# ScuffleCloud/SVT-AV1-mirror

Measured on AMD Instinct MI355X. Metric: open-loop ME 64x64 superblocks/sec + achieved HBM GB/s, 4K preset-8, higher is better.
Workload: dtype u8

## Files before the change

### svt-av1-mirror_amd/csrc/svtme_me_common.h

```cpp
#pragma once
#include <hip/hip_runtime.h>
#include <stdint.h>

#include "svtme_device.h"

#define U32MAX 0xFFFFFFFFu

namespace svtme {

template <typename S, typename T>
__device__ __forceinline__ uint32_t sfld_(const S &obj, const T &f) {
    static_assert(sizeof(T) <= 2 && alignof(S) >= 4, "sfld_: a byte / halfword of a dword-aligned struct");
    const uint32_t off = (uint32_t)((const char *)&f - (const char *)&obj);
    const uint32_t v   = ((const uint32_t *)&obj)[off >> 2] >> (8 * (off & 3));
    return sizeof(T) == 1 ? (v & 0xFFu) : (v & 0xFFFFu);
}
#define SF(obj, field) ::svtme::sfld_((obj), (obj).field)
__device__ __forceinline__ bool tl_or_l0(const svtme_job &j, int l) { return j.temporal_layer_index > 0 || l == 0; }
__device__ __forceinline__ bool slot_valid(uint32_t vmask, int s) { return s >= 0 && s < 8 && ((vmask >> s) & 1u); }
__device__ __forceinline__ uint32_t valid_mask(const svtme_job &job) {
    uint32_t m = 0;
#pragma unroll
    for (int s = 0; s < 8; s++)
        if ((s >> 2) < job.num_lists && (s & 3) < job.num_refs[s >> 2])
            m |= 1u << s;
    return m;
}

#define DPP_ROW_SHR(n) (0x110 + (n))
#define DPP_ROW_BCAST15 0x142
#define DPP_ROW_BCAST31 0x143

template <int CTRL, int RM = 0xF>
__device__ __forceinline__ uint32_t dpp_or(uint32_t v, uint32_t id) {
    return (uint32_t)__builtin_amdgcn_update_dpp((int)id, (int)v, CTRL, RM, 0xF, false);
}
template <typename F>
__device__ __forceinline__ uint32_t wave_scan32(uint32_t v, uint32_t id, F f) {
    v = f(v, dpp_or<DPP_ROW_SHR(1)>(v, id));
    v = f(v, dpp_or<DPP_ROW_SHR(2)>(v, id));
    v = f(v, dpp_or<DPP_ROW_SHR(4)>(v, id));
    v = f(v, dpp_or<DPP_ROW_SHR(8)>(v, id));
    v = f(v, dpp_or<DPP_ROW_BCAST15, 0xA>(v, id));
    v = f(v, dpp_or<DPP_ROW_BCAST31, 0xC>(v, id));
    return v;
}
__device__ __forceinline__ uint32_t lane63(uint32_t v) { return (uint32_t)__builtin_amdgcn_readlane((int)v, 63); }

__device__ __forceinline__ unsigned long long wave_min_u64(unsigned long long v) {
    auto step = [&](uint32_t tl, uint32_t th) {
        const unsigned long long t = ((unsigned long long)th << 32) | tl;
        v                          = t < v ? t : v;
    };
#define WMIN64(CTRL, RM)                                                                                              \
    step(dpp_or<CTRL, RM>((uint32_t)v, U32MAX), dpp_or<CTRL, RM>((uint32_t)(v >> 32), U32MAX))
    WMIN64(DPP_ROW_SHR(1), 0xF);
    WMIN64(DPP_ROW_SHR(2), 0xF);
    WMIN64(DPP_ROW_SHR(4), 0xF);
    WMIN64(DPP_ROW_SHR(8), 0xF);
    WMIN64(DPP_ROW_BCAST15, 0xA);
    WMIN64(DPP_ROW_BCAST31, 0xC);
#undef WMIN64
    return ((unsigned long long)lane63((uint32_t)(v >> 32)) << 32) | lane63((uint32_t)v);
}
__device__ __forceinline__ uint32_t wave_min_u32(uint32_t v) {
    return lane63(wave_scan32(v, U32MAX, [](uint32_t a, uint32_t b) { return a < b ? a : b; }));
}
__device__ __forceinline__ uint32_t wave_sum_u32(uint32_t v) {
    return lane63(wave_scan32(v, 0u, [](uint32_t a, uint32_t b) { return a + b; }));
}
__device__ __forceinline__ int wave_compact(bool pred, int *total) {
    const unsigned long long m = __ballot(pred);
    *total                     = __popcll(m);
    const int lane             = threadIdx.x & 63;
    const unsigned long long lt = lane ? (m & ((1ull << lane) - 1ull)) : 0ull;
    return __popcll(lt);
}

__device__ __forceinline__ int wave_incl_scan(int v) {
    return (int)wave_scan32((uint32_t)v, 0u, [](uint32_t a, uint32_t b) { return a + b; });
}

__device__ __forceinline__ uint32_t magic_u32(uint32_t d) { return 0xFFFFFFFFu / d + 1u; }
__device__ __forceinline__ int mdiv(int n, uint32_t m) { return m ? (int)__umulhi((uint32_t)n, m) : n; }

__device__ __forceinline__ uint32_t xcd_remap(uint32_t bid, uint32_t nwg) {
    const uint32_t xcd = bid & 7, q8 = nwg >> 3, r8 = nwg & 7;
    return (xcd < r8 ? xcd * (q8 + 1) : r8 * (q8 + 1) + (xcd - r8) * q8) + (bid >> 3);
}

#define UNI(x) __builtin_amdgcn_readfirstlane((int)(x))
__device__ __forceinline__ uint32_t rl32(uint32_t v, int l) { return (uint32_t)__builtin_amdgcn_readlane((int)v, l); }
__device__ __forceinline__ uint64_t rl64(uint64_t v, int l) {
    return ((uint64_t)rl32((uint32_t)(v >> 32), l) << 32) | rl32((uint32_t)v, l);
}

template <typename T>
__device__ __forceinline__ T *uni_ptr(T *p) {
    const uint64_t v  = (uint64_t)(uintptr_t)p;
    const uint32_t lo = __builtin_amdgcn_readfirstlane((uint32_t)v);
    const uint32_t hi = __builtin_amdgcn_readfirstlane((uint32_t)(v >> 32));
    return (T *)(uintptr_t)(((uint64_t)hi << 32) | lo);
}

__device__ __forceinline__ unsigned long long qsad(uint32_t lo, uint32_t hi, uint32_t s, unsigned long long a) {
    return __builtin_amdgcn_qsad_pk_u16_u8(((unsigned long long)hi << 32) | lo, s, a);
}
__device__ __forceinline__ void qsad_unpack(unsigned long long a, uint32_t acc[4]) {
    acc[0] += (uint32_t)a & 0xFFFFu;
    acc[1] += (uint32_t)a >> 16;
    acc[2] += (uint32_t)(a >> 32) & 0xFFFFu;
    acc[3] += (uint32_t)(a >> 48);
}

template <int CTRL, int RM = 0xF>
__device__ __forceinline__ uint32_t dpp_add(uint32_t v) {
    return v + (uint32_t)__builtin_amdgcn_update_dpp(0, (int)v, CTRL, RM, 0xF, false);
}

template <int CTRL, int RM = 0xF>
__device__ __forceinline__ uint32_t dpp_add2(uint32_t a, uint32_t b) {
    return a + (uint32_t)__builtin_amdgcn_update_dpp(0, (int)b, CTRL, RM, 0xF, false);
}

__device__ void prehme_area(const DevPlane &p, int16_t org_x, int16_t org_y, int16_t sa_w, int16_t sa_h, int16_t *oxo,
                            int16_t *oyo, int16_t *saw, int16_t *sah) {
    const int16_t pad_w = i16(p.pad - 1), pad_h = i16(p.pad - 1);
    const int16_t pw = i16(p.width), ph = i16(p.height);
    int16_t ox = -(int16_t)(sa_w >> 1);
    int16_t oy = -(int16_t)(sa_h >> 1);
    ox   = ((org_x + ox) < -pad_w) ? i16(-pad_w - org_x) : ox;
    sa_w = ((org_x + ox) < -pad_w) ? i16(sa_w - (-pad_w - (org_x + ox))) : sa_w;
    ox   = ((org_x + ox) > pw - 1) ? i16(ox - ((org_x + ox) - (pw - 1))) : ox;
    sa_w = ((org_x + ox + sa_w) > pw) ? i16(max(1, sa_w - ((org_x + ox + sa_w) - pw))) : sa_w;
    oy   = ((org_y + oy) < -pad_h) ? i16(-pad_h - org_y) : oy;
    sa_h = ((org_y + oy) < -pad_h) ? i16(sa_h - (-pad_h - (org_y + oy))) : sa_h;
    oy   = ((org_y + oy) > ph - 1) ? i16(oy - ((org_y + oy) - (ph - 1))) : oy;
    sa_h = (org_y + oy + sa_h > ph) ? i16(max(1, sa_h - ((org_y + oy + sa_h) - ph))) : sa_h;
    *oxo = ox, *oyo = oy, *saw = sa_w, *sah = sa_h;
}

__device__ void hme_l0_rect(const svtme_controls &c, const DevPlane &p, int16_t org_x, int16_t org_y, int16_t sa_w,
                            int16_t sa_h, int sr_w, int sr_h, int16_t *oxo, int16_t *oyo, int16_t *saw,
                            int16_t *sah) {
    sa_w = i16((sa_w + 7) & ~0x07);
    const int16_t pad_w = i16(p.pad - 1), pad_h = i16(p.pad - 1);
    const int16_t pw = i16(p.width), ph = i16(p.height);
    const int16_t xd = i16(sa_w * sr_w), yd = i16(sa_h * sr_h);
    int16_t ox = i16(-(int16_t)((sa_w * c.num_hme_sa_w) >> 1) + xd);
    int16_t oy = i16(-(int16_t)((sa_h * c.num_hme_sa_h) >> 1) + yd);
    if ((org_x + ox) < -pad_w) {
        ox   = i16(-pad_w - org_x);
        sa_w = i16(sa_w - (-pad_w - (org_x + ox)));
    }
    if ((org_x + ox) > pw - 1)
        ox = i16(ox - ((org_x + ox) - (pw - 1)));
    if ((org_x + ox + sa_w) > pw)
        sa_w = i16(max(1, sa_w - ((org_x + ox + sa_w) - pw)));
    sa_w = (sa_w < 8) ? sa_w : i16(sa_w & ~0x07);
    if ((org_y + oy) < -pad_h) {
        oy   = i16(-pad_h - org_y);
        sa_h = i16(sa_h - (-pad_h - (org_y + oy)));
    }
    if ((org_y + oy) > ph - 1)
        oy = i16(oy - ((org_y + oy) - (ph - 1)));
    if ((org_y + oy + sa_h) > ph)
        sa_h = i16(max(1, sa_h - ((org_y + oy + sa_h) - ph)));
// ... 61 lines not shown
```

### svt-av1-mirror_amd/csrc/svtme_stages.hip

```cpp
#include <hip/hip_ext.h>
#include <cstdlib>
#include <type_traits>

#include "svtme_launch.h"
#include "svtme_me_common.h"

namespace svtme {


#define STAGE_A_BUF_DW 1024
#define STAGE_B_BUF_DW 640

template <int ND, typename P>
__device__ __forceinline__ void rows_qsad(P rp, int bstride_dw, const uint8_t *src, int src_stride,
                                          int k0, int k1, uint32_t acc[4]) {
    constexpr int CH = 64 / ND;
    for (int kc = k0; kc < k1; kc += CH) {
        const int ke         = min(k1, kc + CH);
        unsigned long long a = 0;
#pragma unroll 2
        for (int k = kc; k < ke; k++) {
            const P rd         = rp + k * bstride_dw;
            const uint32_t *sd = (const uint32_t *)(src + k * src_stride);
            uint32_t d[ND + 1];
// ... 887 lines not shown
        if (tk) {
            if (hk) {
                scx = cx;
                scy = cy;
            }
        } else {
            scx = 0;
            scy = 0;
        }
        if (s == k) {
            my_scx = scx, my_scy = scy, my_hs = cs;
        }
    }
    uint64_t hsad = U32MAX;
    if (valid)
        hsad = my_hs;
    uint32_t rdiv = 1;
    uint8_t dref  = s < 8 ? dref0 : 0;
    if (hme_on && !mctf) {
        if (prune && pth != 0xFFFFu) {
            const uint64_t best = wave_min_u64(s < 8 ? hsad : ~0ull);
            if (s < 8 && (s & 3) >= 1 && (hsad - best) * 100 > (pth * best))
                dref = 0;
        }
        if (sradj && s < 8) {
            if (absi(my_scx) <= mvlen && absi(my_scy) <= mvlen && hsad < stat_th)
                rdiv = stat_div;
            else if (hsad < low_th)
                rdiv = low_div;
        }
    }
    SlotCentre o;
    o.hme_sad    = hsad;
    o.zz         = s < 8 ? zz0 : U32MAX;
    o.reduce_div = rdiv;
    o.sc_x       = valid ? my_scx : 0;
    o.sc_y       = valid ? my_scy : 0;
    o.do_ref     = dref;
    return o;
}

#ifndef HME_STAMP
#define HME_STAMP(k)
#endif
#ifndef HME_STOP
#define HME_STOP(k)
#endif
#ifndef HME_SUB
#define HME_SUB(k)
#endif
#ifndef HME_WAVE
#define HME_WAVE(k)
#endif

#define HQ 2
#define HQ1 2
#define HQ16 2

typedef uint32_t u32x4a4 __attribute__((ext_vector_type(4), aligned(4)));
__device__ __forceinline__ u32x4a4 ldg4(const uint32_t *p) {
    typedef __attribute__((address_space(1))) const u32x4a4 gu4;
    return *(gu4 *)(uintptr_t)p;
}
__device__ __forceinline__ __amdgpu_buffer_rsrc_t plane_rsrc(const void *base) {
    return __builtin_amdgcn_make_buffer_rsrc(const_cast<void *>(base), 0, (int)0xFFFFFFFF, 0x00020000);
}
__device__ __forceinline__ u32x4a4 bld4(__amdgpu_buffer_rsrc_t r, uint32_t voff, uint32_t soff) {
    const auto v = __builtin_amdgcn_raw_buffer_load_b128(r, (int)voff, (int)soff, 0);
    u32x4a4 o;
    o.x = v[0], o.y = v[1], o.z = v[2], o.w = v[3];
    return o;
}
__device__ __forceinline__ uint4 sld4(const uint8_t *p) {
    typedef __attribute__((address_space(4))) const uint32_t cu32;
    cu32 *q = (cu32 *)(uintptr_t)p;
    return make_uint4(q[0], q[1], q[2], q[3]);
}
__device__ __forceinline__ unsigned long long qsad64(unsigned long long ref, uint32_t s, unsigned long long a) {
    return __builtin_amdgcn_qsad_pk_u16_u8(ref, s, a);
}
__device__ __forceinline__ unsigned long long pair(uint32_t lo, uint32_t hi) {
    return ((unsigned long long)hi << 32) | lo;
}

struct HSrch {
    const uint8_t *a0;
    int32_t item0;
    int16_t sa_w, ncols;
    int16_t cnt0, cnt1;
    int16_t ylast;
    uint32_t ncm;
    uint8_t sh, skip, id;
    uint8_t need;
    uint8_t tt;
};
struct HSrch1 {
    const uint8_t *a0;
    int32_t item0;
    uint32_t ncm;
    int16_t sa_w, ncols;
    uint8_t sh, id;
};


typedef uint32_t u32x2a4 __attribute__((ext_vector_type(2), aligned(4)));
struct Row8 {
    u32x4a4 lo;
    u32x2a4 hi;
};
__device__ __forceinline__ Row8 row8(const uint8_t *a0, int stride, int ro, int q0) {
    typedef __attribute__((address_space(1))) const u32x2a4 gu2;
    const uint32_t *rp = (const uint32_t *)(a0 + (ptrdiff_t)ro * stride) + q0;
    return Row8{ldg4(rp), *(gu2 *)(uintptr_t)(rp + 4)};
}

template <int T, bool FULLK = false>
__device__ __forceinline__ unsigned long long hme_tile16(const uint8_t *a0, int stride, int q0, int sh, int sa_w,
                                                         int yf, int tv, int ylast, int kh,
                                                         const uint32_t (&sr)[8][4]) {
    constexpr int NR = T + 7;
    kh = UNI(kh);
    unsigned long long acc[T][HQ16];
#pragma unroll
    for (int t = 0; t < T; t++)
#pragma unroll
        for (int qq = 0; qq < HQ16; qq++) acc[t][qq] = 0;
    Row8 buf[3];
    buf[0] = row8(a0, stride, min(yf, ylast), q0);
    buf[1] = row8(a0, stride, min(yf + 2, ylast), q0);
#pragma unroll
    for (int m = 0; m < NR; m++) {
        if (m + 2 < NR)
            buf[(m + 2) % 3] = row8(a0, stride, min(yf + 2 * (m + 2), ylast), q0);
        const Row8 &R = buf[m % 3];
        static_assert(HQ16 + 4 == 6, "Row8 holds 6 dwords");
        const uint32_t d[6] = {R.lo.x, R.lo.y, R.lo.z, R.lo.w, R.hi.x, R.hi.y};
        unsigned long long P[HQ16 + 3];
#pragma unroll
        for (int j = 0; j < HQ16 + 3; j++) P[j] = pair(d[j], d[j + 1]);
#pragma unroll
        for (int t = 0; t < T; t++) {
            const int k = m - t;
            if (k < 0 || k >= 8)
                continue;
            if (!FULLK && k >= kh)
                continue;
#pragma unroll
            for (int qq = 0; qq < HQ16; qq++)
#pragma unroll
                for (int j = 0; j < 4; j++) acc[t][qq] = qsad64(P[qq + j], sr[k][j], acc[t][qq]);
        }
    }
    uint32_t xo[HQ16][4];
#pragma unroll
    for (int qq = 0; qq < HQ16; qq++)
#pragma unroll
        for (int e = 0; e < 4; e++) {
            const int x = 4 * (q0 + qq) - sh + e;
            xo[qq][e]   = (x >= 0 && x < sa_w) ? (uint32_t)x : U32MAX;
        }
    unsigned long long best = ~0ull;
    uint32_t yk = (uint32_t)yf;
    asm volatile("" : "+v"(yk));
#pragma unroll
    for (int t = 0; t < T; t++) {
        uint32_t mt = U32MAX;
#pragma unroll
        for (int qq = 0; qq < HQ16; qq++) {
            const uint32_t lo = (uint32_t)acc[t][qq], hi = (uint32_t)(acc[t][qq] >> 32);
            const uint32_t k0 = (lo << 16) | xo[qq][0], k1 = (lo & 0xFFFF0000u) | xo[qq][1];
            const uint32_t k2 = (hi << 16) | xo[qq][2], k3 = (hi & 0xFFFF0000u) | xo[qq][3];
            mt = min_u32(mt, min_u32(min_u32(k0, k1), min_u32(k2, k3)));
        }
        if (t < tv && mt != U32MAX) {
            const unsigned long long kk = ((unsigned long long)(mt >> 16) << 32) |
                                          ((unsigned long long)(yk + 2 * t) << 16) | (mt & 0xFFFFu);
            best = kk < best ? kk : best;
        }
    }
    return best;
}

template <bool FULLK = false>
__device__ __forceinline__ unsigned long long hme_tile32q(const uint8_t *a0, int stride, int q0, int sh, int sa_w,
                                                          int y, int kh1, const uint8_t (*src)[32]) {
    const int g = threadIdx.x & 3;
    static_assert(HQ1 + 9 == 11, "L1 rows hold 11 dwords");
    typedef uint32_t u32x3a4 __attribute__((ext_vector_type(3), aligned(4)));
    typedef __attribute__((address_space(1))) const u32x3a4 gu3;
    struct Row11 {
        u32x4a4 a, b;
        u32x3a4 c;
    };
    auto ld = [&](int kk, Row11 &L) {
        const int k        = min(4 * g + kk, 15);
        const uint32_t *rp = (const uint32_t *)(a0 + (ptrdiff_t)(y + 2 * k) * stride) + q0;
        L.a = ldg4(rp), L.b = ldg4(rp + 4), L.c = *(gu3 *)(uintptr_t)(rp + 8);
    };
    Row11 L[2];
    ld(0, L[0]);
    unsigned long long acc[HQ1] = {};
#pragma unroll
    for (int kk = 0; kk < 4; kk++) {
        if (kk + 1 < 4)
            ld(kk + 1, L[(kk + 1) & 1]);
        const int k = min(4 * g + kk, 15);
        {
            const Row11 &R = L[kk & 1];
            const uint4 s0 = ((const uint4 *)src[k])[0], s1 = ((const uint4 *)src[k])[1];
            const uint32_t sv[8] = {s0.x, s0.y, s0.z, s0.w, s1.x, s1.y, s1.z, s1.w};
            uint32_t d[11] = {R.a.x, R.a.y, R.a.z, R.a.w, R.b.x, R.b.y, R.b.z, R.b.w, R.c.x, R.c.y, R.c.z};
#pragma unroll
            for (int j = 0; j < HQ1 + 8; j++) d[j] = __builtin_amdgcn_alignbyte(d[j + 1], d[j], (uint32_t)sh);
            const bool use = FULLK || 4 * g + kk < kh1;
#pragma unroll
            for (int qq = 0; qq < HQ1; qq++) {
                unsigned long long a = acc[qq];
#pragma unroll
                for (int j = 0; j < 8; j++) a = qsad64(pair(d[qq + j], d[qq + j + 1]), sv[j], a);
                acc[qq] = use ? a : acc[qq];
            }
        }
    }
    uint32_t mt = U32MAX;
#pragma unroll
    for (int qq = 0; qq < HQ1; qq++) {
        uint32_t a[4] = {0, 0, 0, 0};
        qsad_unpack(acc[qq], a);
#pragma unroll
        for (int e = 0; e < 4; e++) {
            const uint32_t v = dpp_add<0x4E>(dpp_add<0xB1>(a[e]));
            const int x      = 4 * (q0 + qq) + e;
            if (x < sa_w)
                mt = min_u32(mt, (v << 15) | (uint32_t)x);
        }
    }
    if (mt == U32MAX)
        return ~0ull;
    return ((unsigned long long)(mt >> 15) << 32) | ((unsigned long long)(uint32_t)y << 16) | (mt & 0x7FFFu);
}

#define HL2_PITCH 96
__device__ __forceinline__ unsigned long long hme_tile64(const uint8_t *a0, int stride, int q0, int sh, int sa_w,
                                                         int y, int kh2, const uint8_t (*src)[HL2_PITCH]) {
    const int g = threadIdx.x & 7;
    unsigned long long acc[HQ] = {};
#pragma unroll
    for (int kk = 0; kk < 4; kk++) {
        const int k = g + 8 * kk;
        if (k < kh2) {
            const uint32_t *rp = (const uint32_t *)(a0 + (ptrdiff_t)(y + 2 * k) * stride) + q0;
            u32x4a4 L[5];
#pragma unroll
            for (int v = 0; v < 5; v++) L[v] = ldg4(rp + 4 * v);
            uint32_t d[20];
#pragma unroll
            for (int v = 0; v < 5; v++) d[4 * v] = L[v].x, d[4 * v + 1] = L[v].y, d[4 * v + 2] = L[v].z, d[4 * v + 3] = L[v].w;
            constexpr int ND = HQ + 16;
#pragma unroll
            for (int j = 0; j < ND; j++) d[j] = __builtin_amdgcn_alignbyte(d[j + 1], d[j], (uint32_t)sh);
#pragma unroll
            for (int j4 = 0; j4 < 4; j4++) {
                const uint4 sv = ((const uint4 *)src[k])[j4];
                const uint32_t s4[4] = {sv.x, sv.y, sv.z, sv.w};
#pragma unroll
                for (int jj = 0; jj < 4; jj++) {
                    const int j = 4 * j4 + jj;
#pragma unroll
                    for (int qq = 0; qq < HQ; qq++) acc[qq] = qsad64(pair(d[qq + j], d[qq + j + 1]), s4[jj], acc[qq]);
                }
            }
        }
    }
    uint32_t mt = U32MAX;
#pragma unroll
    for (int qq = 0; qq < HQ; qq++) {
        uint32_t a[4] = {0, 0, 0, 0};
        qsad_unpack(acc[qq], a);
#pragma unroll
        for (int e = 0; e < 4; e++) {
            const uint32_t v = dpp_add<0x141>(dpp_add<0x4E>(dpp_add<0xB1>(a[e])));
            const int x      = 4 * (q0 + qq) + e;
            if (x < sa_w)
                mt = min_u32(mt, (v << 13) | (uint32_t)x);
        }
    }
    if (mt == U32MAX)
        return ~0ull;
    return ((unsigned long long)(mt >> 13) << 32) | ((unsigned long long)(uint32_t)y << 16) | (mt & 0x1FFFu);
}

template <typename S>
__device__ __forceinline__ int find_search(const S *t, int n, int it) {
    int lo = 0, hi = n - 1;
    while (lo < hi) {
        const int mid = (lo + hi + 1) >> 1;
        if (t[mid].item0 <= it)
            lo = mid;
        else
            hi = mid - 1;
    }
    return lo;
}

#define HT16 3


struct FpRef {
    const uint32_t *a;
    int32_t sdw;
    int32_t nitems;
    int32_t item_begin;
    uint32_t mnq;
    int16_t xo, yo, w, h;
    int32_t order_base;
    uint8_t slot, nq, sh, pad;
};

// ... 2190 lines not shown
        if (lane < 21)
            decode(lane, sad, mv);
    }
    __syncthreads();
    stage_c_tail<true, NW>(st, dj, sb_local, G.bw, G.bh, vmask);
}

__global__ void __launch_bounds__(256) __attribute__((amdgpu_waves_per_eu(4, 8))) k_stage_e(const DevBatch B) {
    __shared__ StC st;
    uint32_t sb_local;
    const DevJob &dj     = batch_job(B, xcd_remap(blockIdx.x, gridDim.x), &sb_local);
    const SbGeo G        = sb_geo(dj, sb_local);
    const uint32_t vmask = valid_mask(dj.job);
    stage_e_body(st, dj, sb_local, G, vmask, dj.cslot + (size_t)sb_local * dj.R,
                 dj.keys + (size_t)sb_local * dj.R * SVTME_PU_COUNT, dj.parts > 1);
}

struct HmeA {
    Dec d;
    unsigned long long key[SVTME_A_N];
    int16_t kxo[SVTME_A_N], kyo[SVTME_A_N];
    uint32_t need;
    HSrch srch[48];
    int32_t nsrch, nitems;
    int32_t nitems3, base2;
    int32_t end1, base3;
    unsigned long long key1[32];
    int16_t x1o[32], y1o[32];
    HSrch1 s1[32];
    int32_t nsrch1, nitems1;
    int16_t hx[32], hy[32];
    uint64_t hsad[32];
    __attribute__((aligned(16))) uint8_t src4[16][32];
    __attribute__((aligned(16))) uint8_t src1[32][HL2_PITCH];
};

template <int RND>
__device__ __forceinline__ void a1_table(HmeA &A, const DevJob &dj, uint32_t vmask, int16_t sox, int16_t soy, int kh,
                                         uint32_t l0need = 0, int16_t l00x = 0, int16_t l00y = 0,
                                         bool gate = false) {
    const svtme_job &job    = dj.job;
    const svtme_controls &c = job.ctrl;
    const int lane          = threadIdx.x & 63;
    const int s = lane / 6, k = lane - 6 * (lane / 6), l = s >> 2;
    bool on = lane < 48 && slot_valid(vmask, s) && tl_or_l0(job, l) &&
              (k < 2 ? c.prehme_enable != 0 : (c.enable_hme_flag && c.enable_hme_level0_flag));
    if (RND == 1)
        on = on && (k < 2 || s == 0);
    if (RND == 2)
        on = on && k >= 2 && s > 0 && ((l0need >> s) & 1u);
    bool mk    = false;
    int items3 = 0, items2 = 0;
    HSrch e;
    if (on) {
        const DevPlane &P = dj.ref[l][s & 3].lv[2];
        int16_t aw = k < 2 ? dj.ph_sa[s][k][0] : dj.l0_sa[s][0];
        int16_t ah = k < 2 ? dj.ph_sa[s][k][1] : dj.l0_sa[s][1];
        if (RND == 2)
            hme_l0_area(c, l, s & 3, dj.sdist[s], l00x, l00y, &aw, &ah);
        int16_t xo, yo, sw, shh;
        bool skip;
        if (k < 2) {
            prehme_area(P, sox, soy, aw, ah, &xo, &yo, &sw, &shh);
            skip   = c.prehme_skip_search_line != 0;
            e.id   = (uint8_t)(SVTME_A_PH + s * 2 + k);
            e.need = (uint8_t)(s * 2);
        } else {
            hme_l0_rect(c, P, sox, soy, aw, ah, (k - 2) >> 1, (k - 2) & 1, &xo, &yo, &sw, &shh);
            skip   = false;
            e.id   = (uint8_t)(SVTME_A_L0 + s * 4 + (k - 2));
            e.need = (uint8_t)(s * 2 + 1);
        }
        A.kxo[e.id]    = xo;
        A.kyo[e.id]    = yo;
        const int nrows = (sw > 0 && shh > 0) ? (skip ? shh / 2 : shh) : 0;
        if (nrows > 0) {
            const uint8_t *w0 = P.base + (ptrdiff_t)(soy + yo) * P.stride + (sox + xo);
            e.sh              = (uint8_t)((uintptr_t)w0 & 3);
            e.a0              = w0 - e.sh;
            e.sa_w            = sw;
            e.skip            = skip;
            const int nq      = (e.sh + sw + 3) >> 2;
            e.ncols           = (int16_t)((nq + HQ16 - 1) / HQ16);
            e.ncm             = magic_u32((uint32_t)e.ncols);
            if (skip) {
                e.cnt0  = (int16_t)nrows;
                e.cnt1  = 0;
                e.ylast = (int16_t)(2 * nrows - 1 + 2 * (kh - 1));
                items3  = e.ncols * ((nrows + HT16 - 1) / HT16);
                items2  = e.ncols * ((nrows + 1) / 2);
            } else {
                e.cnt0  = (int16_t)((nrows + 1) >> 1);
                e.cnt1  = (int16_t)(nrows >> 1);
                e.ylast = (int16_t)(nrows - 1 + 2 * (kh - 1));
                items3  = e.ncols * 2 * ((e.cnt0 + HT16 - 1) / HT16);
                items2  = e.ncols * 2 * ((e.cnt0 + 1) / 2);
            }
            mk = true;
        }
    }
    const bool l0    = k >= 2;
    const bool g     = RND == 0 && gate && mk && !l0 && l == 1;
    const int n3_pre = (int)wave_sum_u32(mk && !l0 && !g ? (uint32_t)items3 : 0u);
    const int n3_l0  = (int)wave_sum_u32(mk && l0 ? (uint32_t)items3 : 0u);
    const int n2_l0  = (int)wave_sum_u32(mk && l0 ? (uint32_t)items2 : 0u);
    const bool split = ((n3_pre + 63) / 64) * HT16 + ((n2_l0 + 63) / 64) * 2 < ((n3_pre + n3_l0 + 63) / 64) * HT16;
    const bool t2    = mk && split && l0;
    const int items  = t2 ? items2 : items3;
    e.tt             = (uint8_t)(t2 ? 2 : HT16);
    int n3s, n2s, ngs;
    const int k3 = wave_compact(mk && !t2 && !g, &n3s), k2 = wave_compact(t2, &n2s), kg = wave_compact(g, &ngs);
    const int i3 = wave_incl_scan(mk && !t2 && !g ? items : 0), i2 = wave_incl_scan(t2 ? items : 0);
    const int ig = wave_incl_scan(g ? items : 0);
    const int N3 = (int)lane63((uint32_t)i3), N2 = (int)lane63((uint32_t)i2), NG = (int)lane63((uint32_t)ig);
    const int base2 = (N3 + 63) & ~63;
    const int end1  = N2 ? base2 + N2 : N3;
    const int base3 = (end1 + 63) & ~63;
    if (mk) {
        e.item0 = g ? base3 + ig - items : t2 ? base2 + i2 - items : i3 - items;
        A.srch[g ? n3s + n2s + kg : t2 ? n3s + k2 : k3] = e;
    }
    if (lane == 0) {
        A.nsrch   = n3s + n2s + ngs;
        A.nitems3 = N3;
        A.base2   = base2;
        A.end1    = end1;
        A.base3   = NG ? base3 : end1;
        A.nitems  = NG ? base3 + NG : end1;
    }
}

__device__ __forceinline__ bool a1_mirrored(const HmeA &A, const svtme_controls &c, uint32_t need, int id) {
    const int r = ((id - SVTME_A_PH) >> 1) & 3, k = (id - SVTME_A_PH) & 1;
    if (c.me_early_exit_th && A.d.zz[r] < c.me_early_exit_th)
        return true;
    if (!((need >> (2 * r)) & 1u))
        return false;
    const int id0 = SVTME_A_PH + 2 * r + k;
    uint32_t best;
    int x, y;
    key_result(A.key[id0], &best, &x, &y);
    const uint32_t sad = best * 2;
    const int16_t col = i16((x + A.kxo[id0]) * 4), row = i16((y + A.kyo[id0]) * 4);
    return sad < 32 * 32 || (absi(col) < 16 && absi(row) < 16);
}

struct HmeSh {
    DevJob dj;
    BState bs;
    CSlot cin[8];
    SlotCentre cen[8];
    uint8_t tf_exit;
    union U {
        HmeA a;
        StC st;
    } u;
};

#define HME_PRIO_HI() __builtin_amdgcn_s_setprio(2)
#define HME_PRIO_LO() __builtin_amdgcn_s_setprio(0)
#define HME_WAVES_PER_EU 8
template <bool FP, bool SUB_ME, bool K32, bool RT = false, int NW = 4>
__global__ void __launch_bounds__(64 * NW) __attribute__((amdgpu_waves_per_eu(HME_WAVES_PER_EU, HME_WAVES_PER_EU))) k_hme(const DevBatch B) {
    static_assert(NW == 3 || NW == 4, "k_hme: 3 or 4 wavefronts");
    static_assert(sizeof(HmeSh) <= 16384, "HmeSh: ten workgroups per CU (160 KB of LDS)");
    constexpr int NT = 64 * NW;
    __shared__ HmeSh sh;
// ... 92 lines not shown
            }
            const uint32_t best = wave_min_u32(zz);
            if (have && (lane & 3) > 0 && tli > 0 && best < zth && (uint32_t)((zz - best) * 100u) > (uint32_t)(zpct * best))
                dref = false;
            if (slz) {
                const uint32_t z0 = rl32(zz, 0), z4 = rl32(zz, 4);
                const bool safe = hl > 0 && nl == 2 && tli >= hl && sbr && z0 < slz && z4 < slz;
                if (safe && slot_valid(vmask, lane) && (lane & 3) > 0)
                    dref = false;
            }
        }
        if (lane < 8) {
            d.zz[lane]     = zz;
            d.do_ref[lane] = dref ? 1 : 0;
        }
        const int s       = lane >> 1;
        const uint32_t zs = (uint32_t)__builtin_amdgcn_ds_bpermute(4 * s, (int)zz);
        const uint32_t ds = (uint32_t)__builtin_amdgcn_ds_bpermute(4 * s, dref ? 1 : 0);
        const bool act    = lane < 16 && slot_valid(vmask, s) && tl_or_l0(job, s >> 2) && ds;
        const bool nd     = act && ((lane & 1) ? !(eet && zs < (eet >> 2)) : !(eet && zs < eet));
        const unsigned long long m = __ballot(nd);
        if (lane == 0)
            sh.u.a.need = (uint32_t)m;
        HME_PRIO_LO();
    } else if (wid == 1) {
        if (lane < SVTME_A_N)
            sh.u.a.key[lane] = ~0ull;
        const bool gate = !RT && c.prehme_enable && c.prehme_l1_early_exit && job.num_lists == 2 &&
                          c.hme_search_method != SVTME_FULL_SAD_SEARCH && !(dj.paths & SVTME_PATH_NO_A1_GATE);
        a1_table<RT ? 1 : 0>(sh.u.a, dj, vmask, sox, soy, kh, 0, 0, 0, gate);
    } else {
        if (c.enable_hme_level2_flag) {
            const DevPlane &F = dj.cur.lv[0];
            constexpr int NP = 128 / (NT - 128);
            u32x4a4 v[NP];
#pragma unroll
            for (int p = 0; p < NP; p++) {
                const int i = tid - 128 + p * (NT - 128), row = i >> 2, part = i & 3;
                v[p] = ldg4((const uint32_t *)(F.base + (ptrdiff_t)(G.oy + 2 * row) * F.stride + G.ox + 16 * part));
            }
#pragma unroll
            for (int p = 0; p < NP; p++) {
                const int i = tid - 128 + p * (NT - 128), row = i >> 2, part = i & 3;
                ((uint4 *)sh.u.a.src1[row])[part] = make_uint4(v[p].x, v[p].y, v[p].z, v[p].w);
            }
        }
        if (c.enable_hme_level1_flag && tid < 160) {
            const DevPlane &Q = dj.cur.lv[1];
            const int row = (tid - 128) >> 1, half = tid & 1;
            const u32x4a4 v = ldg4((const uint32_t *)(Q.base + (ptrdiff_t)((G.oy >> 1) + 2 * row) * Q.stride +
                                                      (G.ox >> 1) + 16 * half));
            ((uint4 *)sh.u.a.src4[row])[half] = make_uint4(v.x, v.y, v.z, v.w);
        }
    }
    HME_WAVE(0);
    __syncthreads();
    HME_STAMP(1);
    HME_STAMP(2);
    auto a1_tiles = [&]() {
        uint32_t sr[8][4];
        {
            const uint8_t *sp = uni_ptr(dj.cur.lv[2].base + (ptrdiff_t)soy * dj.cur.lv[2].stride + sox);
            const int sst     = UNI(dj.cur.lv[2].stride);
#pragma unroll
            for (int k = 0; k < 8; k++) {
                const uint4 v = sld4(sp + (ptrdiff_t)(2 * k) * sst);
                sr[k][0] = v.x, sr[k][1] = v.y, sr[k][2] = v.z, sr[k][3] = v.w;
            }
        }
        const int nitems = sh.u.a.nitems, nsrch = sh.u.a.nsrch;
        const uint32_t need = sh.u.a.need;
        const int pstride = dj.cur.lv[2].stride;
        const int nitems3 = sh.u.a.nitems3, base2 = sh.u.a.base2, end1 = sh.u.a.end1, base3 = sh.u.a.base3;
        auto tiles = [&](auto fullk, int lo, int hi, bool gated) {
            for (int it = lo + tid; it < hi; it += NT) {
                if (it >= nitems3 && it < base2)
                    continue;
                const HSrch &e = sh.u.a.srch[find_search(sh.u.a.srch, nsrch, it)];
                if (!((need >> e.need) & 1u))
                    continue;
                if (gated && a1_mirrored(sh.u.a, c, need, e.id))
                    continue;
                const int local = it - e.item0;
                const int rt = mdiv(local, e.ncm), col = local - rt * e.ncols;
                auto run = [&](auto TT) {
                    constexpr int T = decltype(TT)::value;
                    int yf, tv;
                    if (e.skip) {
                        yf = 2 * T * rt + 1;
                        tv = min(T, e.cnt0 - T * rt);
                    } else {
                        const int p = rt & 1, i = rt >> 1;
                        yf = 2 * T * i + p;
                        tv = min(T, (p ? e.cnt1 : e.cnt0) - T * i);
                    }
                    if (tv <= 0)
                        return;
                    const unsigned long long kk = hme_tile16<T, decltype(fullk)::value>(
                        e.a0, pstride, HQ16 * col, e.sh, e.sa_w, yf, tv, e.ylast, kh, sr);
                    if (kk != ~0ull)
                        atomicMin(&sh.u.a.key[e.id], kk);
                };
                if (UNI(it >= base2 && it < base3))
                    run(std::integral_constant<int, 2>());
                else
                    run(std::integral_constant<int, HT16>());
            }
        };
        tiles(std::false_type(), 0, end1, false);
        if (base3 < nitems) {
            __syncthreads();
            tiles(std::false_type(), base3, nitems, true);
        }
    };
    a1_tiles();
    if constexpr (RT) {
        __syncthreads();
        if (wid == 0) {
            HME_PRIO_HI();
            if (lane < SVTME_A_N && lane >= SVTME_A_PH) {
                uint32_t best;
                int x, y;
                key_result(sh.u.a.key[lane], &best, &x, &y);
                d.a[lane] = ARes{best * 2, i16((x + sh.u.a.kxo[lane]) * 4),
                                 i16((y + sh.u.a.kyo[lane]) * 4)};
            }
            wave_lds_fence();
            dec_prehme(d, job, vmask);
            dec_l0(d, job, vmask);
            const int s = lane;
            bool run    = s > 0 && s < 8 && slot_valid(vmask, s) && tl_or_l0(job, s >> 2) && d.do_ref[s] &&
                       !(c.me_early_exit_th && d.zz[s] < (c.me_early_exit_th >> 2));
            if (run && c.prev_me_stage_based_exit_th) {
                const int k = d.ph[s][0].sad <= d.ph[s][1].sad ? 0 : 1;
                run = !(d.ph[s][k].performed && d.ph[s][k].sad < (c.prev_me_stage_based_exit_th >> 4));
            }
            const uint32_t l0need = (uint32_t)__ballot(run);
            a1_table<2>(sh.u.a, dj, vmask, sox, soy, kh, l0need, d.lx[0][0], d.ly[0][0]);
            if (lane == 0)
                sh.u.a.need = ~0u;
        }
        __syncthreads();
        HME_PRIO_LO();
        a1_tiles();
    }
    __syncthreads();
    HME_STAMP(3);
    const bool hsub = c.hme_search_method != SVTME_FULL_SAD_SEARCH;
    if (wid == 0) {
        HME_PRIO_HI();
        const int mlane = (int)__builtin_amdgcn_mbcnt_hi(~0u, __builtin_amdgcn_mbcnt_lo(~0u, 0u));
        const int s = mlane >> 2, q = mlane & 3, l = s >> 2;
        int16_t X0 = 0, Y0 = 0;
        uint32_t S0 = 0, zzs, drs;
        if constexpr (RT) {
            if (lane < SVTME_A_N && lane >= SVTME_A_PH) {
                uint32_t best;
                int x, y;
                key_result(sh.u.a.key[lane], &best, &x, &y);
                d.a[lane] = ARes{hsub ? best * 2 : best, i16((x + sh.u.a.kxo[lane]) * 4), i16((y + sh.u.a.kyo[lane]) * 4)};
            }
            wave_lds_fence();
            dec_l0(d, job, vmask);
            if (lane < 32) {
                X0 = d.lx[s][q], Y0 = d.ly[s][q], S0 = (uint32_t)d.lsad[s][q];
            }
            zzs = d.zz[s & 7], drs = d.do_ref[s & 7];
// ... 61 lines not shown
                const bool bperf  = (k1 ? f1 : f0) != 0;
                uint32_t kb;
                int kx, ky;
                key_result(kl0, &kb, &kx, &ky);
                if (sv) {
                    if (eet && zzs < (eet >> 2)) {
                    } else if (pmse && bperf && bs < (pmse >> 4)) {
                        X0 = (int16_t)(bcr & 0xFFFFu), Y0 = (int16_t)(bcr >> 16), S0 = bs;
                    } else if (!drs) {
                        S0 = U32MAX;
                    } else if (tl) {
                        X0   = i16((kx + lxo) * 4);
                        Y0   = i16((ky + lyo) * 4);
                        S0   = hsub ? kb * 2 : kb;
                        srch = true;
                    }
                }
                const unsigned long long sm = __ballot(srch);
                if (ph_on && lane < 32 && ((sm >> (4 * s)) & 0xFu)) {
                    const uint32_t q0 = dpp_or<0x00>(S0, 0u), q1 = dpp_or<0x55>(S0, 0u);
                    const uint32_t q2 = dpp_or<0xAA>(S0, 0u), q3 = dpp_or<0xFF>(S0, 0u);
                    int wq = 0;
                    uint32_t mx = 0;
                    if (q0 > mx) { mx = q0; wq = 0; }
                    if (q2 > mx) { mx = q2; wq = 2; }
                    if (q1 > mx) { mx = q1; wq = 1; }
                    if (q3 > mx) { wq = 3; }
                    const uint32_t sw = wq == 0 ? q0 : wq == 1 ? q1 : wq == 2 ? q2 : q3;
                    if (q == wq && bs < sw) {
                        S0 = bs;
                        X0 = (int16_t)(bcr & 0xFFFFu);
                        Y0 = (int16_t)(bcr >> 16);
                    }
                }
            }
            if (lane < 32) {
                d.lx[s][q]   = X0;
                d.ly[s][q]   = Y0;
                d.lsad[s][q] = S0;
            }
            if (lane < 32 && q == 0)
                d.do_ref[s] = (uint8_t)drs;
        }
        bool mk   = false;
        int items = 0;
        HSrch1 e;
        if (lane < 32) {
            int16_t X = 0, Y = 0;
            uint64_t SD = 0;
            sh.u.a.key1[lane] = ~0ull;
            const bool listed = c.enable_hme_flag && c.enable_hme_level1_flag && slot_valid(vmask, s) &&
                                tl_or_l0(job, l);
            if (listed) {
                bool done = false;
                if (c.me_early_exit_th && zzs < (c.me_early_exit_th >> 2)) {
                    X = Y = 0;
                    SD   = 0;
                    done = true;
                }
                if (!done && !drs) {
                    X = Y = 0;
                    SD   = U32MAX;
                    done = true;
                }
                if (!done && c.prev_me_stage_based_exit_th && S0 < (c.prev_me_stage_based_exit_th >> 5)) {
                    X = X0, Y = Y0, SD = S0;
                    done = true;
                }
                if (!done) {
                    const DevPlane &P = dj.ref[l][s & 3].lv[1];
                    const int16_t qx = i16(((int16_t)G.ox) >> 1), qy = i16(((int16_t)G.oy) >> 1);
                    int16_t xo, yo, sw, shh;
                    hme_refine_rect(1, P, qx, qy, (int16_t)c.hme_l1_sa.width, (int16_t)c.hme_l1_sa.height,
                                    i16(X0 >> 1), i16(Y0 >> 1), &xo, &yo, &sw, &shh);
                    sh.u.a.x1o[lane] = xo;
                    sh.u.a.y1o[lane] = yo;
                    SD           = ~0ull;
                    if (sw > 0 && shh > 0 && kh1 > 0) {
                        const uint8_t *w0 = P.base + (ptrdiff_t)(qy + yo) * P.stride + (qx + xo);
                        e.sh              = (uint8_t)((uintptr_t)w0 & 3);
                        e.a0              = w0 - e.sh;
                        e.sa_w            = sw;
                        e.ncols           = (int16_t)((((sw + 3) >> 2) + HQ1 - 1) / HQ1);
                        e.ncm             = magic_u32((uint32_t)e.ncols);
                        e.id              = (uint8_t)lane;
                        items             = e.ncols * shh;
                        mk                = true;
                    }
                }
            }
            sh.u.a.hx[lane]   = X;
            sh.u.a.hy[lane]   = Y;
            sh.u.a.hsad[lane] = SD;
        }
        int tot;
        const int kpos = wave_compact(mk, &tot);
        const int incl = wave_incl_scan(items);
        if (mk) {
            e.item0     = incl - items;
            sh.u.a.s1[kpos] = e;
        }
        if (lane == 63)
            sh.u.a.nitems1 = incl;
        if (lane == 0)
            sh.u.a.nsrch1 = tot;
    }
    __syncthreads();
    HME_PRIO_LO();
    HME_STAMP(4);
    {
        const int nlanes = 4 * sh.u.a.nitems1, nsrch = sh.u.a.nsrch1;
        const int pstride = dj.cur.lv[1].stride;
        auto tiles = [&](auto fullk) {
            for (int it4 = tid; it4 < nlanes; it4 += NT) {
                const int it    = it4 >> 2;
                const HSrch1 &e = sh.u.a.s1[find_search(sh.u.a.s1, nsrch, it)];
                const int local = it - e.item0;
                const int y = mdiv(local, e.ncm), col = local - y * e.ncols;
                const unsigned long long kk = hme_tile32q<decltype(fullk)::value>(e.a0, pstride, HQ1 * col, e.sh,
                                                                                  e.sa_w, y, kh1, sh.u.a.src4);
                if ((it4 & 3) == 0 && kk != ~0ull)
                    atomicMin(&sh.u.a.key1[e.id], kk);
            }
        };
        tiles(std::false_type());
    }
    __syncthreads();
    if (wid == 0 && lane < 32 && sh.u.a.hsad[lane] == ~0ull) {
        uint32_t best;
        int x, y;
        key_result(sh.u.a.key1[lane], &best, &x, &y);
        sh.u.a.hsad[lane] = hsub ? (uint64_t)best * 2 : best;
        sh.u.a.hx[lane]   = i16((x + sh.u.a.x1o[lane]) * 2);
        sh.u.a.hy[lane]   = i16((y + sh.u.a.y1o[lane]) * 2);
    }
    if (c.enable_hme_level2_flag) {
        if (wid == 0) {
            const int s = lane >> 2, l = s >> 2;
            bool mk   = false;
            int items = 0;
            HSrch1 e;
            if (lane < 32) {
                sh.u.a.key1[lane] = ~0ull;
                const bool listed = c.enable_hme_flag && slot_valid(vmask, s) && tl_or_l0(job, l);
                const bool keep   = c.prev_me_stage_based_exit_th &&
                                  sh.u.a.hsad[lane] < (c.prev_me_stage_based_exit_th >> 2);
                if (listed && !keep) {
                    const DevPlane &P = dj.ref[l][s & 3].lv[0];
                    int16_t xo, yo, sw, shh;
                    hme_refine_rect(2, P, (int16_t)G.ox, (int16_t)G.oy, (int16_t)c.hme_l2_sa.width,
                                    (int16_t)c.hme_l2_sa.height, sh.u.a.hx[lane], sh.u.a.hy[lane], &xo, &yo, &sw, &shh);
                    sh.u.a.x1o[lane]  = xo;
                    sh.u.a.y1o[lane]  = yo;
                    sh.u.a.hsad[lane] = ~0ull;
                    if (sw > 0 && shh > 0) {
                        const uint8_t *w0 = P.base + (ptrdiff_t)((int16_t)G.oy + yo) * P.stride + ((int16_t)G.ox + xo);
                        e.sh              = (uint8_t)((uintptr_t)w0 & 3);
                        e.a0              = w0 - e.sh;
                        e.sa_w            = sw;
                        e.ncols           = (int16_t)((((sw + 3) >> 2) + HQ - 1) / HQ);
                        e.ncm             = magic_u32((uint32_t)e.ncols);
                        e.id              = (uint8_t)lane;
                        items             = e.ncols * shh;
                        mk                = true;
                    }
                }
            }
            int tot;
            const int kpos = wave_compact(mk, &tot);
            const int incl = wave_incl_scan(items);
            if (mk) {
                e.item0            = incl - items;
                sh.u.a.s1[kpos] = e;
            }
            if (lane == 63)
                sh.u.a.nitems1 = incl;
            if (lane == 0)
                sh.u.a.nsrch1 = tot;
        }
        __syncthreads();
        {
            const int nlanes = 8 * sh.u.a.nitems1, nsrch = sh.u.a.nsrch1;
            const int pstride = dj.cur.lv[0].stride;
            const int kh2     = (int)(G.bh >> 1);
            for (int it8 = tid; it8 < nlanes; it8 += NT) {
                const int it    = it8 >> 3;
                const HSrch1 &e = sh.u.a.s1[find_search(sh.u.a.s1, nsrch, it)];
                const int local = it - e.item0;
                const int y = mdiv(local, e.ncm), col = local - y * e.ncols;
                const unsigned long long kk = hme_tile64(e.a0, pstride, HQ * col, e.sh, e.sa_w, y, kh2, sh.u.a.src1);
                if ((it8 & 7) == 0 && kk != ~0ull)
                    atomicMin(&sh.u.a.key1[e.id], kk);
            }
        }
        __syncthreads();
        if (wid == 0 && lane < 32 && sh.u.a.hsad[lane] == ~0ull) {
            uint32_t best;
            int x, y;
            key_result(sh.u.a.key1[lane], &best, &x, &y);
            sh.u.a.hsad[lane] = hsub ? (uint64_t)best * 2 : best;
            sh.u.a.hx[lane]   = i16(x + sh.u.a.x1o[lane]);
            sh.u.a.hy[lane]   = i16(y + sh.u.a.y1o[lane]);
        }
    }
    HME_STAMP(5);
    BState *b = FP ? &sh.bs : dj.bst + sb_local;
    if (wid == 0) {
        if (lane < 32) {
            b->hx[0][lane]         = sh.u.a.hx[lane];
            b->hy[0][lane]         = sh.u.a.hy[lane];
            b->hsad[0][lane]       = sh.u.a.hsad[lane];
            (&b->lx[0][0])[lane]   = (&d.lx[0][0])[lane];
            (&b->ly[0][0])[lane]   = (&d.ly[0][0])[lane];
            (&b->lsad[0][0])[lane] = (&d.lsad[0][0])[lane];
        }
        if (lane < 8) {
            b->zz[lane]     = d.zz[lane];
            b->do_ref[lane] = d.do_ref[lane];
        }
    }
    if (!FP) {
        HME_STAMP(6);
        return;
    }
    if (wid == 0) {
        HME_PRIO_HI();
        wave_lds_fence();
        const SlotCentre scv = final_centre(gj.job, &sh.bs, vmask);
        if (lane < 8)
            sh.cen[lane] = scv;
        if (lane == 0)
            sh.tf_exit = job.me_type == SVTME_ME_MCTF && scv.hme_sad < job.tf_me_exit_th;
    }
    __syncthreads();
    HME_PRIO_LO();
    HME_STOP(55);
    const int nrec = (int)dj.R, nr0 = (int)SF(gj.job, num_refs[0]);
    const uint8_t tfx = (uint8_t)UNI(sh.tf_exit);
    for (int k = 0, j = 0; k < nrec; k++) {
        constexpr int ROWS = SUB_ME ? 4 : 8, RSTEP = SUB_ME ? 2 : 1;
        const int s         = k < nr0 ? k : 4 + (k - nr0);
        const SlotCentre &v = sh.cen[s];
        const bool srch     = UNI(v.do_ref) && !tfx;
        const int owner     = srch ? j : NW - 1;
        j                   = srch ? (j + 1 == NW ? 0 : j + 1) : j;
        if (wid != owner)
            continue;
        if (!srch) {
            if (lane == 0)
                sh.cin[k] = fp_unsearched(v.hme_sad, v.zz, v.sc_x, v.sc_y, v.do_ref, tfx);
            continue;
        }
        int fl = lane;
        asm volatile("" : "+v"(fl));
        const int z16 = fl >> 2, k4 = fl & 3;
        const int by  = ((z16 >> 3) << 2) | (((z16 >> 1) & 1) << 1) | (k4 >> 1);
        const int bx  = (((z16 >> 2) & 1) << 2) | ((z16 & 1) << 1) | (k4 & 1);
        const DevPlane &C = gj.cur.lv[0];
        const int cst     = UNI(C.stride);
        const __amdgpu_buffer_rsrc_t crs = plane_rsrc(uni_ptr(C.base + (ptrdiff_t)G.oy * cst + G.ox));
        const uint32_t coff = (uint32_t)(by * 8 * cst + bx * 8);
        uint32_t src[ROWS][2];
#pragma unroll
        for (int rr = 0; rr < ROWS; rr++) {
            const auto v = __builtin_amdgcn_raw_buffer_load_b64(crs, (int)coff, rr * RSTEP * cst, 0);
            src[rr][0] = v[0];
            src[rr][1] = v[1];
        }
        fp_slot<SUB_ME, K32, 2, false, HME_WHOLE>(gj, G, s, src, by, bx, rl64(v.hme_sad, 0), (uint32_t)UNI(v.zz), (uint32_t)UNI(v.reduce_div),
                                (int16_t)UNI(v.sc_x), (int16_t)UNI(v.sc_y), (uint8_t)UNI(v.do_ref), tfx, 0, 1u,
                                &sh.u.st.keys[k][0], &sh.cin[k]);
    }
// ... 80 lines not shown
```

Measured before the change: 72.74 million.

## Trim ALU work in HME tile SAD kernels: pair packing, interior fast path, float division

Builds the odd 64-bit qsad operand pairs from neighbouring even pairs using v_pk_mov_b32 with op_sel, so fewer pair-building moves are issued. Adds a wave-uniform interior fast path that skips per-position bounds masks in the tile reductions. In hme_tile32q it hoists the row address arithmetic, drops the row clamp, and adds a fast path for full kh1 height. It also moves the dpp reduction ahead of the bounds checks. Magic-multiply division is replaced by a float reciprocal multiply, which is cheaper but relies on float precision holding exactly for the index ranges seen. Removing the min(...,15) clamp could change behaviour if kh1 ever exceeds the tile rows.

```diff
diff --git a/svt-av1-mirror_amd/csrc/svtme_me_common.h b/svt-av1-mirror_amd/csrc/svtme_me_common.h
--- a/svt-av1-mirror_amd/csrc/svtme_me_common.h
+++ b/svt-av1-mirror_amd/csrc/svtme_me_common.h
@@ -83,6 +83,8 @@
 
 __device__ __forceinline__ uint32_t magic_u32(uint32_t d) { return 0xFFFFFFFFu / d + 1u; }
 __device__ __forceinline__ int mdiv(int n, uint32_t m) { return m ? (int)__umulhi((uint32_t)n, m) : n; }
+__device__ __forceinline__ float rdiv_of(int d) { return __builtin_amdgcn_rcpf((float)d); }
+__device__ __forceinline__ int rdiv(int n, float r) { return (int)(((float)n + 0.5f) * r); }
 
 __device__ __forceinline__ uint32_t xcd_remap(uint32_t bid, uint32_t nwg) {
     const uint32_t xcd = bid & 7, q8 = nwg >> 3, r8 = nwg & 7;
diff --git a/svt-av1-mirror_amd/csrc/svtme_stages.hip b/svt-av1-mirror_amd/csrc/svtme_stages.hip
--- a/svt-av1-mirror_amd/csrc/svtme_stages.hip
+++ b/svt-av1-mirror_amd/csrc/svtme_stages.hip
@@ -993,6 +993,11 @@
 __device__ __forceinline__ unsigned long long pair(uint32_t lo, uint32_t hi) {
     return ((unsigned long long)hi << 32) | lo;
 }
+__device__ __forceinline__ unsigned long long pair_hi_lo(unsigned long long a, unsigned long long b) {
+    unsigned long long r;
+    asm("v_pk_mov_b32 %0, %1, %2 op_sel:[1,0]" : "=v"(r) : "v"(a), "v"(b));
+    return r;
+}
 
 struct HSrch {
     const uint8_t *a0;
@@ -1000,7 +1005,7 @@
     int16_t sa_w, ncols;
     int16_t cnt0, cnt1;
     int16_t ylast;
-    uint32_t ncm;
+    float ncr;
     uint8_t sh, skip, id;
     uint8_t need;
     uint8_t tt;
@@ -1008,7 +1013,7 @@
 struct HSrch1 {
     const uint8_t *a0;
     int32_t item0;
-    uint32_t ncm;
+    float ncr;
     int16_t sa_w, ncols;
     uint8_t sh, id;
 };
@@ -1048,7 +1053,9 @@
         const uint32_t d[6] = {R.lo.x, R.lo.y, R.lo.z, R.lo.w, R.hi.x, R.hi.y};
         unsigned long long P[HQ16 + 3];
 #pragma unroll
-        for (int j = 0; j < HQ16 + 3; j++) P[j] = pair(d[j], d[j + 1]);
+        for (int j = 0; j < HQ16 + 3; j += 2) P[j] = pair(d[j], d[j + 1]);
+#pragma unroll
+        for (int j = 1; j < HQ16 + 3; j += 2) P[j] = pair_hi_lo(P[j - 1], P[j + 1]);
 #pragma unroll
         for (int t = 0; t < T; t++) {
             const int k = m - t;
@@ -1062,32 +1069,46 @@
                 for (int j = 0; j < 4; j++) acc[t][qq] = qsad64(P[qq + j], sr[k][j], acc[t][qq]);
         }
     }
-    uint32_t xo[HQ16][4];
-#pragma unroll
-    for (int qq = 0; qq < HQ16; qq++)
-#pragma unroll
-        for (int e = 0; e < 4; e++) {
-            const int x = 4 * (q0 + qq) - sh + e;
-            xo[qq][e]   = (x >= 0 && x < sa_w) ? (uint32_t)x : U32MAX;
-        }
+    const int x0 = 4 * q0 - sh;
+    const bool inner = __builtin_amdgcn_ballot_w64(x0 < 0 || x0 + 4 * HQ16 > sa_w) == 0;
     unsigned long long best = ~0ull;
     uint32_t yk = (uint32_t)yf;
     asm volatile("" : "+v"(yk));
-#pragma unroll
-    for (int t = 0; t < T; t++) {
-        uint32_t mt = U32MAX;
-#pragma unroll
-        for (int qq = 0; qq < HQ16; qq++) {
-            const uint32_t lo = (uint32_t)acc[t][qq], hi = (uint32_t)(acc[t][qq] >> 32);
-            const uint32_t k0 = (lo << 16) | xo[qq][0], k1 = (lo & 0xFFFF0000u) | xo[qq][1];
-            const uint32_t k2 = (hi << 16) | xo[qq][2], k3 = (hi & 0xFFFF0000u) | xo[qq][3];
-            mt = min_u32(mt, min_u32(min_u32(k0, k1), min_u32(k2, k3)));
-        }
-        if (t < tv && mt != U32MAX) {
-            const unsigned long long kk = ((unsigned long long)(mt >> 16) << 32) |
-                                          ((unsigned long long)(yk + 2 * t) << 16) | (mt & 0xFFFFu);
-            best = kk < best ? kk : best;
-        }
+    auto rows = [&](auto in, const uint32_t (&xo)[HQ16][4]) {
+        constexpr bool IN = decltype(in)::value;
+#pragma unroll
+        for (int t = 0; t < T; t++) {
+            uint32_t mt = U32MAX;
+#pragma unroll
+            for (int qq = 0; qq < HQ16; qq++) {
+                const uint32_t lo = (uint32_t)acc[t][qq], hi = (uint32_t)(acc[t][qq] >> 32);
+                const uint32_t k0 = (lo << 16) | xo[qq][0], k1 = (lo & 0xFFFF0000u) | xo[qq][1];
+                const uint32_t k2 = (hi << 16) | xo[qq][2], k3 = (hi & 0xFFFF0000u) | xo[qq][3];
+                mt = min_u32(mt, min_u32(min_u32(k0, k1), min_u32(k2, k3)));
+            }
+            if (IN)
+                mt += (uint32_t)x0;
+            if (t < tv && (IN || mt != U32MAX)) {
+                const unsigned long long kk = ((unsigned long long)(mt >> 16) << 32) |
+                                              ((unsigned long long)(yk + 2 * t) << 16) | (mt & 0xFFFFu);
+                best = kk < best ? kk : best;
+            }
+        }
+    };
+    if (inner) {
+        static_assert(HQ16 == 2, "a tile's 8 positions");
+        const uint32_t xe[HQ16][4] = {{0, 1, 2, 3}, {4, 5, 6, 7}};
+        rows(std::true_type(), xe);
+    } else {
+        uint32_t xo[HQ16][4];
+#pragma unroll
+        for (int qq = 0; qq < HQ16; qq++)
+#pragma unroll
+            for (int e = 0; e < 4; e++) {
+                const int x = x0 + 4 * qq + e;
+                xo[qq][e]   = (x >= 0 && x < sa_w) ? (uint32_t)x : U32MAX;
+            }
+        rows(std::false_type(), xo);
     }
     return best;
 }
@@ -1103,19 +1124,21 @@
         u32x4a4 a, b;
         u32x3a4 c;
     };
+    const int st2      = 2 * UNI(stride);
+    const uint8_t *rp0 = a0 + (ptrdiff_t)(y + 8 * g) * stride + 4 * q0;
     auto ld = [&](int kk, Row11 &L) {
-        const int k        = min(4 * g + kk, 15);
-        const uint32_t *rp = (const uint32_t *)(a0 + (ptrdiff_t)(y + 2 * k) * stride) + q0;
+        const uint32_t *rp = (const uint32_t *)(rp0 + (ptrdiff_t)(kk * st2));
         L.a = ldg4(rp), L.b = ldg4(rp + 4), L.c = *(gu3 *)(uintptr_t)(rp + 8);
     };
     Row11 L[2];
     ld(0, L[0]);
+    const bool fullh = UNI(kh1) == 16;
     unsigned long long acc[HQ1] = {};
 #pragma unroll
     for (int kk = 0; kk < 4; kk++) {
         if (kk + 1 < 4)
             ld(kk + 1, L[(kk + 1) & 1]);
-        const int k = min(4 * g + kk, 15);
+        const int k = 4 * g + kk;
         {
             const Row11 &R = L[kk & 1];
             const uint4 s0 = ((const uint4 *)src[k])[0], s1 = ((const uint4 *)src[k])[1];
@@ -1123,28 +1146,57 @@
             uint32_t d[11] = {R.a.x, R.a.y, R.a.z, R.a.w, R.b.x, R.b.y, R.b.z, R.b.w, R.c.x, R.c.y, R.c.z};
 #pragma unroll
             for (int j = 0; j < HQ1 + 8; j++) d[j] = __builtin_amdgcn_alignbyte(d[j + 1], d[j], (uint32_t)sh);
-            const bool use = FULLK || 4 * g + kk < kh1;
+            static_assert(HQ1 + 8 == 10, "pairs 0 .. 8 of 10 realigned dwords");
+            unsigned long long P[HQ1 + 7];
+#pragma unroll
+            for (int j = 0; j < HQ1 + 7; j += 2) P[j] = pair(d[j], d[j + 1]);
+#pragma unroll
+            for (int j = 1; j < HQ1 + 7; j += 2) P[j] = pair_hi_lo(P[j - 1], P[j + 1]);
+            unsigned long long a[HQ1];
 #pragma unroll
             for (int qq = 0; qq < HQ1; qq++) {
-                unsigned long long a = acc[qq];
-#pragma unroll
-                for (int j = 0; j < 8; j++) a = qsad64(pair(d[qq + j], d[qq + j + 1]), sv[j], a);
-                acc[qq] = use ? a : acc[qq];
-            }
-        }
+                a[qq] = acc[qq];
+#pragma unroll
+                for (int j = 0; j < 8; j++) a[qq] = qsad64(P[qq + j], sv[j], a[qq]);
+            }
+            if (!FULLK && !fullh) {
+                const bool use = k < kh1;
+#pragma unroll
+                for (int qq = 0; qq < HQ1; qq++) {
+                    uint32_t lo = use ? (uint32_t)a[qq] : (uint32_t)acc[qq];
+                    uint32_t hi = use ? (uint32_t)(a[qq] >> 32) : (uint32_t)(acc[qq] >> 32);
+                    asm volatile("" : "+v"(lo), "+v"(hi));
+                    a[qq] = pair(lo, hi);
+                }
+            }
+#pragma unroll
+            for (int qq = 0; qq < HQ1; qq++) acc[qq] = a[qq];
+        }
+    }
+    uint32_t v[HQ1][4];
+#pragma unroll
+    for (int qq = 0; qq < HQ1; qq++) {
+        const uint32_t lo = dpp_add<0xB1>((uint32_t)acc[qq]), hi = dpp_add<0xB1>((uint32_t)(acc[qq] >> 32));
+        v[qq][0] = dpp_add<0x4E>(lo & 0xFFFFu), v[qq][1] = dpp_add<0x4E>(lo >> 16);
+        v[qq][2] = dpp_add<0x4E>(hi & 0xFFFFu), v[qq][3] = dpp_add<0x4E>(hi >> 16);
     }
     uint32_t mt = U32MAX;
-#pragma unroll
-    for (int qq = 0; qq < HQ1; qq++) {
-        uint32_t a[4] = {0, 0, 0, 0};
-        qsad_unpack(acc[qq], a);
-#pragma unroll
-        for (int e = 0; e < 4; e++) {
-            const uint32_t v = dpp_add<0x4E>(dpp_add<0xB1>(a[e]));
-            const int x      = 4 * (q0 + qq) + e;
-            if (x < sa_w)
-                mt = min_u32(mt, (v << 15) | (uint32_t)x);
-        }
+    static_assert(HQ1 == 2, "a tile's 8 positions: x = 8 * column + 0 .. 7");
+    if (__builtin_amdgcn_ballot_w64(4 * (q0 + HQ1) > sa_w) == 0) {
+#pragma unroll
+        for (int qq = 0; qq < HQ1; qq++)
+#pragma unroll
+            for (int e = 0; e < 4; e++) mt = min_u32(mt, (v[qq][e] << 15) | (uint32_t)(4 * qq + e));
+        mt |= (uint32_t)(4 * q0);
+    } else {
+#pragma unroll
+        for (int qq = 0; qq < HQ1; qq++)
+#pragma unroll
+            for (int e = 0; e < 4; e++) {
+                const int x = 4 * (q0 + qq) + e;
+                if (x < sa_w)
+                    mt = min_u32(mt, (v[qq][e] << 15) | (uint32_t)x);
+            }
     }
     if (mt == U32MAX)
         return ~0ull;
@@ -3501,7 +3553,7 @@
             e.skip            = skip;
             const int nq      = (e.sh + sw + 3) >> 2;
             e.ncols           = (int16_t)((nq + HQ16 - 1) / HQ16);
-            e.ncm             = magic_u32((uint32_t)e.ncols);
+            e.ncr             = rdiv_of(e.ncols);
             if (skip) {
                 e.cnt0  = (int16_t)nrows;
                 e.cnt1  = 0;
@@ -3760,7 +3812,7 @@
                 if (gated && a1_mirrored(sh.u.a, c, need, e.id))
                     continue;
                 const int local = it - e.item0;
-                const int rt = mdiv(local, e.ncm), col = local - rt * e.ncols;
+                const int rt = rdiv(local, e.ncr), col = local - rt * e.ncols;
                 auto run = [&](auto TT) {
                     constexpr int T = decltype(TT)::value;
                     int yf, tv;
@@ -3988,7 +4040,7 @@
                         e.a0              = w0 - e.sh;
                         e.sa_w            = sw;
                         e.ncols           = (int16_t)((((sw + 3) >> 2) + HQ1 - 1) / HQ1);
-                        e.ncm             = magic_u32((uint32_t)e.ncols);
+                        e.ncr             = rdiv_of(e.ncols);
                         e.id              = (uint8_t)lane;
                         items             = e.ncols * shh;
                         mk                = true;
@@ -4022,7 +4074,7 @@
                 const int it    = it4 >> 2;
                 const HSrch1 &e = sh.u.a.s1[find_search(sh.u.a.s1, nsrch, it)];
                 const int local = it - e.item0;
-                const int y = mdiv(local, e.ncm), col = local - y * e.ncols;
+                const int y = rdiv(local, e.ncr), col = local - y * e.ncols;
                 const unsigned long long kk = hme_tile32q<decltype(fullk)::value>(e.a0, pstride, HQ1 * col, e.sh,
                                                                                   e.sa_w, y, kh1, sh.u.a.src4);
                 if ((it4 & 3) == 0 && kk != ~0ull)
@@ -4065,7 +4117,7 @@
                         e.a0              = w0 - e.sh;
                         e.sa_w            = sw;
                         e.ncols           = (int16_t)((((sw + 3) >> 2) + HQ - 1) / HQ);
-                        e.ncm             = magic_u32((uint32_t)e.ncols);
+                        e.ncr             = rdiv_of(e.ncols);
                         e.id              = (uint8_t)lane;
                         items             = e.ncols * shh;
                         mk                = true;
@@ -4093,7 +4145,7 @@
                 const int it    = it8 >> 3;
                 const HSrch1 &e = sh.u.a.s1[find_search(sh.u.a.s1, nsrch, it)];
                 const int local = it - e.item0;
-                const int y = mdiv(local, e.ncm), col = local - y * e.ncols;
+                const int y = rdiv(local, e.ncr), col = local - y * e.ncols;
                 const unsigned long long kk = hme_tile64(e.a0, pstride, HQ * col, e.sh, e.sa_w, y, kh2, sh.u.a.src1);
                 if ((it8 & 7) == 0 && kk != ~0ull)
                     atomicMin(&sh.u.a.key1[e.id], kk);
```

New measurement: 74.21 million, median of 6. 2.0% higher.
